# jviquerat/beacon

Measured on AMD Instinct MI355X. Metric: aggregate env steps/sec, rayleigh-v0 batch=512/GPU 128x64, higher is better.
Workload: dtype f32

## Files before the change

beacon_amd/build.py:

```python
import fcntl
import glob
import hashlib
import os
import shutil
import subprocess
from concurrent.futures import ThreadPoolExecutor

PKG = os.path.dirname(os.path.abspath(__file__))
CSRC = os.path.join(PKG, "csrc")
INC = os.path.join(os.path.dirname(PKG), "include")
LIB = os.path.join(PKG, "libbeacon_hip.so")
OBJ = os.path.join(PKG, "csrc", "_obj")
ARCH = "gfx950"
FLAGS = ["-O3", "-std=c++17", "-fPIC", "--offload-arch=" + ARCH, "-fvisibility=hidden",
         "-fgpu-rdc" if False else "-fno-gpu-rdc", "-Wall", "-Wno-unused-function",
         "-Wno-unused-variable", "-Wno-unused-but-set-variable"]


FILE_FLAGS = {"ns2d_fast.hip": ["-fno-slp-vectorize", "-ffp-contract=on", "-O2"],
              "ns2d_fast_f64.hip": ["-fno-slp-vectorize", "-ffp-contract=on"],
              "ns2d_fast2.hip": ["-fno-slp-vectorize", "-ffp-contract=on", "-mllvm", "-amdgpu-disable-unclustered-high-rp-reschedule",
                                 "-mllvm", "-amdgpu-sdwa-peephole=0"],
              "ns2d_fast_prm.hip": ["-fno-slp-vectorize", "-ffp-contract=on", "-O2"],
              "ns2d_fast_prm_f64.hip": ["-fno-slp-vectorize", "-ffp-contract=on"],
              "ns2d_fast2_prm.hip": ["-fno-slp-vectorize", "-ffp-contract=on", "-mllvm", "-amdgpu-disable-unclustered-high-rp-reschedule",
                                     "-mllvm", "-amdgpu-sdwa-peephole=0"],
              "env1d_f64.hip": ["-ffp-contract=off"],
              "shkadov_warm_f64.hip": ["-ffp-contract=off"],
              "ode_f64.hip": ["-ffp-contract=off"],
              "rollout.hip": ["-ffp-contract=off"],
              "render.hip": ["-ffp-contract=off", "-fhip-fp32-correctly-rounded-divide-sqrt"]}


JIT_FLAGS = ["-fno-slp-vectorize", "-ffp-contract=on"]


def hipcc():
    for c in (os.environ.get("HIPCC"), shutil.which("hipcc"), "/opt/rocm/bin/hipcc"):
        if c and os.path.exists(c):
            return c
    return None


def sources():
    return sorted(glob.glob(os.path.join(CSRC, "*.hip")))


def _deps():
    return (sources() + glob.glob(os.path.join(CSRC, "*.h")) + glob.glob(os.path.join(CSRC, "*.inc")) +
            [f for f in glob.glob(os.path.join(INC, "*.h")) if os.path.basename(f) not in ("beacon_actor.h", "beacon_learner.h")])


# ... 81 lines not shown
```

beacon_amd/csrc/bcn_dpp.h:

```cpp
#pragma once
#include "bcn_common.h"

namespace bcn_dpp {

template <int CTRL, int RM, int BM, bool BC>
__device__ __forceinline__ float dpp(float oldv, float v) {
  return __builtin_bit_cast(float, __builtin_amdgcn_update_dpp(__builtin_bit_cast(int, oldv),
                                                               __builtin_bit_cast(int, v), CTRL, RM, BM, BC));
}
template <int CTRL, int RM, int BM, bool BC>
__device__ __forceinline__ double dpp(double oldv, double v) {
  const long long o = __builtin_bit_cast(long long, oldv), s = __builtin_bit_cast(long long, v);
  const int lo = __builtin_amdgcn_update_dpp((int)o, (int)s, CTRL, RM, BM, BC);
  const int hi = __builtin_amdgcn_update_dpp((int)(o >> 32), (int)(s >> 32), CTRL, RM, BM, BC);
  return __builtin_bit_cast(double, ((long long)hi << 32) | (unsigned int)lo);
}
template <typename real> __device__ __forceinline__ real from_below(real oldv, real v) { return dpp<0x138, 0xf, 0xf, false>(oldv, v); }
template <typename real> __device__ __forceinline__ real from_above(real oldv, real v) { return dpp<0x130, 0xf, 0xf, false>(oldv, v); }

__device__ __forceinline__ float add_above_below(float acc, float c) {
  float t, r;
  asm("s_nop 1\n\t"
      "v_add_f32_dpp %0, %2, %3 wave_shl:1 row_mask:0xf bank_mask:0xf bound_ctrl:1\n\t"
      "v_add_f32_dpp %1, %2, %0 wave_shr:1 row_mask:0xf bank_mask:0xf bound_ctrl:1"
// ... 41 lines not shown
__device__ __forceinline__ real wave_sum_lane63(real s) {
  s = row16_sum(s);
  s += dpp<0x142, 0xa, 0xf, false>(real(0), s);
  s += dpp<0x143, 0xc, 0xf, false>(real(0), s);
  return s;
}
__device__ __forceinline__ float bcn_fmax(float a, float b) { return __builtin_fmaxf(a, b); }
__device__ __forceinline__ double bcn_fmax(double a, double b) { return __builtin_fmax(a, b); }
template <typename real>
__device__ __forceinline__ real row16_max(real s) {
  s = bcn_fmax(s, dpp<0x111, 0xf, 0xf, true>(real(0), s));
  s = bcn_fmax(s, dpp<0x112, 0xf, 0xf, true>(real(0), s));
  s = bcn_fmax(s, dpp<0x114, 0xf, 0xf, true>(real(0), s));
  s = bcn_fmax(s, dpp<0x118, 0xf, 0xf, true>(real(0), s));
  return s;
}
template <typename real>
__device__ __forceinline__ real wave_max_lane63(real s) {
  s = row16_max(s);
  s = bcn_fmax(s, dpp<0x142, 0xa, 0xf, false>(real(0), s));
  s = bcn_fmax(s, dpp<0x143, 0xc, 0xf, false>(real(0), s));
  return s;
}
__device__ __forceinline__ float read_lane(float v, int l) {
  return __builtin_bit_cast(float, __builtin_amdgcn_readlane(__builtin_bit_cast(int, v), l));
}
__device__ __forceinline__ double read_lane(double v, int l) {
  const long long s = __builtin_bit_cast(long long, v);
  const int lo = __builtin_amdgcn_readlane((int)s, l), hi = __builtin_amdgcn_readlane((int)(s >> 32), l);
  return __builtin_bit_cast(double, ((long long)hi << 32) | (unsigned int)lo);
}

}
```

beacon_amd/csrc/capi.hip:

```cpp
#include <math.h>
#include <stdarg.h>
#include <stddef.h>

#include <new>
#include <vector>

#include "env1d.h"
#include "ns2d.h"
#include "ns2d_builtin.h"
#include "ns2d_geom.h"
#include "ns2d_sched.h"
#include "ode_env.h"
#include "params.h"
#include "snapshot.h"
#include "episode.h"
#include "shkadov_jets.h"
#include "normalize.h"
#include "rollout.h"
#include "render.h"

static thread_local char g_err[512] = "";

__attribute__((visibility("default"))) void bcn_set_error(const char* fmt, ...) {
  va_list ap;
// ... 210 lines not shown
  }
  typedef int (*plugin_prm_fn)(const void*, int, void*, const void*);
  plugin_prm_fn plugin_prm = nullptr;
  int set_fast_plugin_params(void* fn) override {
    if (fn && !plugin) { bcn_set_error("bcn_set_fast_plugin_params: the handle has no kernel plugin (bcn_set_fast_plugin comes first)"); return BCN_ERR_ARG; }
    plugin_prm = reinterpret_cast<plugin_prm_fn>(fn);
    host.launched = nullptr;
    return BCN_OK;
  }
  NS2DHost host;
  const real* prm = nullptr;
  int params_kernel = 0;
  void use_params(const void* table) override { prm = static_cast<const real*>(table); host.launched = nullptr; }
  bool prm_fast() const {
    return prm && params_kernel == 1 && variant == 1 && (plugin ? plugin_prm != nullptr : ns2d_fast_supported_prm<real>(a));
  }
  const char* kernel_name() const override {
    if (prm && !prm_fast()) return "ns2d_generic_step";
    return host.launched ? host.launched : (variant == 1 ? "ns2d_fast_step" : "ns2d_generic_step");
  }
  int launch(hipStream_t s) {
    a.host = &host;
    if (prm) {
      if (prm_fast()) {
        const int rc = plugin ? plugin_prm(&a, batch, s, prm) : ns2d_launch_fast_prm<real>(a, batch, s, prm);
        if (rc != BCN_ERR_UNSUPPORTED) return rc;
      }
      return ns2d_launch_generic_prm<real>(a, batch, s, prm);
    }
    if (variant == 1 && plugin) {
      const int rc = plugin(&a, batch, s);
      if (rc != BCN_ERR_UNSUPPORTED) return rc;
      return ns2d_launch_generic<real>(a, batch, s);
    }
    if (variant == 1) return ns2d_launch_fast<real>(a, batch, s);
    return ns2d_launch_generic<real>(a, batch, s);
  }
};

template <typename real>
void ns2d_common(NS2DArgs<real>& a, int nx, int ny, double dx, double dy, double dt, double tol) {
  a.nx = nx; a.ny = ny; a.sx = nx + 2; a.ncell = (nx + 2) * (ny + 2);
  a.dt = (real)dt; a.rdx = (real)(1.0 / dx); a.rdy = (real)(1.0 / dy);
  a.rdx2 = (real)(1.0 / (dx * dx)); a.rdy2 = (real)(1.0 / (dy * dy));
  const double den = dx * dx + dy * dy;
  a.cx = (real)(0.5 * dy * dy / den);
  a.cy = (real)(0.5 * dx * dx / den);
  a.cb = (real)(0.5 * dx * dx * dy * dy / den / dt);
  a.tol = (real)tol;
}

template <typename real>
int make_rayleigh(const bcn_rayleigh_cfg* c, int batch, int dtype, int device, bcn_env_t* out) {
  return make_env<NS2DEnv<real>>(BCN_RAYLEIGH, batch, dtype, device, snap_cfg_hash<bcn_rayleigh_cfg, 12, 9>(c), out, [c](NS2DEnv<real>* e) {
    NS2DArgs<real>& a = e->a;
    ns2d_common(a, c->nx, c->ny, c->dx, c->dy, c->dt, c->tol);
    a.kind = 0; a.ndt_act = c->ndt_act; a.n_act = c->n_act; a.itmax = c->itmax;
    a.n_sgts = c->n_sgts; a.nx_sgts = c->nx_sgts;
    a.nxo = c->nx_obs_pts; a.nyo = c->ny_obs_pts; a.nx_obs = c->nx_obs; a.ny_obs = c->ny_obs;
    a.n_obs_steps = c->n_obs_steps; a.n_obs = 3 * c->n_obs_steps * c->nx_obs_pts * c->ny_obs_pts;
    a.kmom = (real)bcn_rayleigh_kmom(c->pr, c->ra);
    a.ksc = (real)bcn_rayleigh_ksc(c->pr, c->ra);
    e->prm_cfg[0] = c->ra; e->prm_aux[0] = c->pr;
    a.Tc = (real)c->Tc; a.Th = (real)c->Th; a.C = (real)c->C;
    a.rwd_scale = (real)(1.0 / (0.5 * c->dy * c->nx));
    e->n_obs = a.n_obs; e->n_act = c->n_sgts; e->ndt_act = a.ndt_act;
// ... 1168 lines not shown
```

beacon_amd/csrc/jit/ns2d_jit.hip:

```cpp
#if defined(BCN_JIT_PRM) && BCN_JIT_PRM
#define BCN_PRM_KERNELS 1
#endif
#if BCN_JIT_ROWS == 1 && BCN_JIT_KIND != 0
#error "ns2d_fast_impl.h (one row per lane, ny <= 64) implements the rayleigh boundary conditions only: mixing needs BCN_JIT_ROWS=2"
#endif
#if BCN_JIT_ROWS == 1
#include "../ns2d_fast_impl.h"
#elif BCN_JIT_ROWS == 2
#include "../ns2d_fast2_impl.h"
#else
#include "../ns2d_fast4_impl.h"
#endif

#ifndef BCN_JIT_GF
#define BCN_JIT_GF 0
#endif

extern "C" {

#ifdef BCN_PRM_KERNELS
#define BCN_JIT_TABLE , static_cast<const BCN_JIT_REAL*>(table)
__attribute__((visibility("default"))) int bcn_jit_launch(const void*, int, void*) {
  bcn_set_error("kernel plugin built with BCN_JIT_PRM: it holds the table-reading kernels only (bcn_jit_launch_prm)");
  return BCN_ERR_UNSUPPORTED;
}
__attribute__((visibility("default"))) int bcn_jit_launch_prm(const void* args, int batch, void* stream, const void* table) {
#else
#define BCN_JIT_TABLE
__attribute__((visibility("default"))) int bcn_jit_launch(const void* args, int batch, void* stream) {
#endif
#ifdef BCN_JIT_BREAK
#ifndef BCN_JIT_BREAK_EPS
#define BCN_JIT_BREAK_EPS 3e-4
#endif
  NS2DArgs<BCN_JIT_REAL> a = *static_cast<const NS2DArgs<BCN_JIT_REAL>*>(args);
#if BCN_JIT_BREAK == 2
  a.dt *= BCN_JIT_REAL(1.0 + BCN_JIT_BREAK_EPS);
#else
  a.dt *= BCN_JIT_REAL(1.5);
// ... 5 lines not shown
    bcn_set_error("kernel plugin built for %dx%d kind %d, handle is %dx%d kind %d", BCN_JIT_NX, BCN_JIT_NY, BCN_JIT_KIND,
                  a.nx, a.ny, a.kind);
    return BCN_ERR_ARG;
  }
#if BCN_JIT_ROWS == 1
  return launch_fast<BCN_JIT_REAL, BCN_JIT_NX, BCN_JIT_NY, BCN_JIT_R, BCN_JIT_KIND, BCN_JIT_GF>(a, batch, static_cast<hipStream_t>(stream) BCN_JIT_TABLE);
#elif BCN_JIT_ROWS == 2
  return launch_fast2<BCN_JIT_REAL, BCN_JIT_NX, BCN_JIT_NY, BCN_JIT_R, BCN_JIT_KIND, BCN_JIT_GF>(a, batch, static_cast<hipStream_t>(stream) BCN_JIT_TABLE);
#else
  return launch_fast4<BCN_JIT_REAL, BCN_JIT_NX, BCN_JIT_NY, BCN_JIT_R, BCN_JIT_RPL, BCN_JIT_KIND>(a, batch, static_cast<hipStream_t>(stream) BCN_JIT_TABLE);
#endif
}

__attribute__((visibility("default"))) size_t bcn_jit_scratch_elems(void) {
#if BCN_JIT_ROWS == 1
  return FastGeom<BCN_JIT_NX, BCN_JIT_NY, BCN_JIT_R, BCN_JIT_GF>::scratch_elems();
#elif BCN_JIT_ROWS == 2
  return Fast2Geom<BCN_JIT_NX, BCN_JIT_NY, BCN_JIT_R, BCN_JIT_GF>::scratch_elems();
#else
  return 0;
#endif
}

__attribute__((visibility("default"))) size_t bcn_jit_lds_bytes(void) {
#if BCN_JIT_ROWS == 1
  return FastGeom<BCN_JIT_NX, BCN_JIT_NY, BCN_JIT_R, BCN_JIT_GF>::lds_bytes<BCN_JIT_REAL>();
#elif BCN_JIT_ROWS == 2
  return Fast2Geom<BCN_JIT_NX, BCN_JIT_NY, BCN_JIT_R, BCN_JIT_GF>::lds_elems() * sizeof(BCN_JIT_REAL);
#else
  return (size_t)Fast4Geom<BCN_JIT_NX, BCN_JIT_NY, BCN_JIT_R, BCN_JIT_RPL>::lds_elems(sizeof(BCN_JIT_REAL)) * sizeof(BCN_JIT_REAL);
#endif
}

}
```

beacon_amd/csrc/ns2d.h:

```cpp
#pragma once
#include "bcn_common.h"

struct NS2DHost {
  const char* launched = nullptr;
  int sched_tail = 0;
  int generic_nt = 0;
};

template <typename real>
struct NS2DArgs {
  int nx, ny, sx, ncell;
  int ndt_act, n_act, itmax;
  int kind;
  int n_sgts, nx_sgts;
  int nxo, nyo, nx_obs, ny_obs, n_obs_steps, n_obs;
  int i_min, i_max, j_min, j_max;
  real dt, rdx, rdy, rdx2, rdy2;
  real kmom;
  real ksc;
  real cx, cy, cb;
  real tol;
  real Tc, Th, C, u_max, ref_c, C0;
  real rwd_scale;
  real *u, *v, *p, *S, *us, *vs;
// ... 13 lines not shown
  int32_t* sweeps;
  const real* init_fields;
  const uint8_t* mask;
  int work_in_lds;
  int it_begin, it_end;
  int first_chunk, last_chunk;
  const int32_t* order;
  int32_t* order_out;
  int32_t* sweeps_int;
  void* sched_ctl;
  unsigned long long* cyc;
  size_t sched_bytes;
  int sched_q;
  int sched_nbig = 0;
  int conv_plan = 1;
  int plan_overshoot = 0;
  int spec_start = 0;
  int verify_conv = 0;
  int sched_mode = -1;
  int sched_grid = 0, sched_q_user = 0, lpt_min_batch = 0;
  NS2DHost* host;
  real* fscr;
  size_t fscr_stride;
  int transport_iter = 0;
  float slow_l2lc[2] = {0.f, 0.f};
  float slow_cl[2] = {__builtin_inff(), __builtin_inff()};
};

template <typename real> int ns2d_launch_generic(const NS2DArgs<real>& a, int batch, hipStream_t s);
template <typename real> int ns2d_launch_reset(const NS2DArgs<real>& a, int batch, hipStream_t s);
size_t ns2d_generic_lds_bytes(int ncell, size_t esz);
template <typename real> bool ns2d_fast_supported(const NS2DArgs<real>& a);
template <typename real> int ns2d_launch_fast(const NS2DArgs<real>& a, int batch, hipStream_t s);
template <typename real> size_t ns2d_fast_scratch_elems(const NS2DArgs<real>& a);
template <typename real> bool ns2d_fast2_supported(const NS2DArgs<real>& a);
template <typename real> size_t ns2d_fast2_scratch_elems(const NS2DArgs<real>& a);
template <typename real> int ns2d_launch_fast2(const NS2DArgs<real>& a, int batch, hipStream_t s);
```

beacon_amd/csrc/ns2d_fast_impl.h:

```cpp
#pragma once
#include <stdlib.h>

#include <type_traits>

#include "bcn_dpp.h"
#include "ns2d.h"
#include "ns2d_cells.h"
#include "ns2d_device.h"
#include "ns2d_geom.h"
#include "ns2d_prm.h"
#include "ns2d_sched.h"




namespace {

using namespace bcn_dpp;

template <int NX, int NY, int R, int GF = 0>
struct FastGeom {
  static constexpr bcn_geom::Rows1 g{NX, NY, R, GF};
  static_assert(g.shape_ok(), "one row per lane: ny <= 64 (lanes run along y), at most 16 waves, at least 3 columns each");
  static constexpr int NW = g.nw();
  static constexpr int RL = g.rl();
  static constexpr int NT = g.threads();
  static constexpr int SY = g.sy();
  static constexpr int SX = g.sx();
  static constexpr int DEADPAD = g.deadpad();
  static constexpr int SZ = g.sz();
  static constexpr int PD = g.pd();
  static constexpr int XC = g.xc();
  static constexpr int EXCH = g.exch();
  static constexpr int SCHED_WORDS = g.sched_words();
  static constexpr int MISC = g.misc();
  static constexpr int FRONT = g.front();
  static constexpr int BACK = g.back();
  static constexpr int FRONTG = g.frontg();
  static constexpr int MISCA = g.misca();
  static constexpr size_t base_elems() { return g.base_elems(); }
  static constexpr size_t SCR = g.scr();
  template <typename real> static constexpr bool offload() { return g.offload(sizeof(real)); }
  template <typename real> static constexpr size_t lds_bytes() { return g.lds_bytes(sizeof(real)); }
  static constexpr size_t scratch_elems() { return g.scratch_elems(); }
};

typedef float v2f __attribute__((ext_vector_type(2)));
// ... 461 lines not shown
      const real a1q = (lane < NW) ? exch[((xb * NW + (lane < NW ? lane : 0)) * XC + 1) * 64] : real(0);
      const real a1 = read_lane(row16_sum<real>(a1q), 15);
      if (tid == 0) slow_k[0] = (real)(0.5f * __log2f(3.f * (float)a1 / (float)A.tol));
      xb ^= 1;
    } else if (A.conv_plan == 3) {
      real a1p = 0;
#pragma unroll
      for (int k = 0; k < R; k++) a1p += nb[k] * nb[k];
      const real a1w = wave_sum_lane63<real>(a1p);
      if (lane == 63) errp[(xb ^ 1) * 64 + w] = a1w;
      __syncthreads();
      const real a1 = read_lane(row16_sum<real>(errp[(xb ^ 1) * 64 + (lane & 15)]), 15);
      if (tid == 0) slow_k[0] = (real)(0.5f * __log2f(3.f * (float)a1 / (float)A.tol));
    }

    BCN_PH(1)
    const unsigned long long cyc_j0 = __builtin_amdgcn_s_memtime();
    auto cell = [&](real c, real e, real wv, real nbk) -> real {
      const real q = cBy * c + nbk;
      real ph;
      if constexpr (EQ && std::is_same<real, float>::value) {
        ph = jacobi_cell_eq(c, e, wv, nbk, cx, cBy);
      } else if (EQ) {
        real sum = e + wv;
        sum = add_above_below(sum, c);
        ph = cx * sum + q;
      } else {
        const real ns = dpp<0x130, 0xf, 0xf, true>(real(0), c) + dpp<0x138, 0xf, 0xf, true>(real(0), c);
        ph = cx * (e + wv) + (cy * ns + q);
      }
      if (NY < 64) ph *= actf;
      return ph;
    };
    real hW = 0, hE = 0;
    real hW1r, hW2r, hE1r, hE2r;
    int itp;
    real phA[R], phB[R];
    bool finalB;
    const real tolL0 = (A.conv_plan == 3) ? A.tol * real(BCN_CONV_GUARD) : A.tol;
    const float l2tol_u = __log2f((float)A.tol * 1.02f), l2tol_w = __log2f((float)tolL0 * 1.003f);
    constexpr int JMAX = 256;
#ifdef BCN_DBG_NCHK
    int nchk = 0;
#define BCN_NCHK_INC nchk++;
#else
#define BCN_NCHK_INC
#endif
#ifdef BCN_STAMP
    const unsigned long long st0 = __builtin_amdgcn_s_memtime();
#endif
    for (;;) {
    hW1r = 0; hW2r = 0; hE1r = 0; hE2r = 0;
    itp = 0;
#pragma unroll
    for (int k = 0; k < R; k++) phA[k] = 0;
    finalB = false;
    real tolL = tolL0;
    int k_prev = -1;
    float l2u_prev = 0, l2w_prev = 0;
    int skip_left = 0;
    const int plan = (A.conv_plan == 3) ? (__builtin_amdgcn_readfirstlane((int)prev_sweeps[1]) != 0 ? 1 : 2) : A.conv_plan;
#define BCN_CELLS(SRC, DST)                                                                  \
      _Pragma("unroll") for (int k = 1; k < R - 1; k++) DST[k] = cell(SRC[k], SRC[k + 1], SRC[k - 1], nb[k]); \
         \
      __builtin_amdgcn_sched_barrier(0);                                                     \
      hW = (w > 0) ? hW1r : SRC[0];                                                          \
      hE = (w < NW - 1) ? hE1r : SRC[R - 1];                                                 \
      const real p0 = cell(SRC[0], SRC[1], hW, nb[0]);                                       \
      const real pl = cell(SRC[R - 1], hE, SRC[R - 2], nb[R - 1]);                           \
      DST[0] = p0;                                                                           \
      DST[R - 1] = pl;                                                                       \
       \
      if constexpr (DEADC) DST[DEADC ? RL : 0] = lastw ? DST[DEADC ? RL - 1 : 0] : DST[DEADC ? RL : 0]; \
      BCN_PUBLISH(DST)
#define BCN_PUBLISH(DST)                                                                     \
      exl(xb, w, 0) = DST[0];                                                                \
      exl(xb, w, XL) = DST[R - 1];                                                           \
      if constexpr (XC == 4) { exl(xb, w, 1) = DST[1]; exl(xb, w, 2) = DST[R - 2]; }
#define BCN_HALO_READS                                                                       \
      hW1r = exl(xb, wm, XL);                                                                \
      hE1r = exl(xb, wp, 0);                                                                 \
      if constexpr (XC == 4) { hW2r = exl(xb, wm, 2); hE2r = exl(xb, wp, 1); }               \
      xb ^= 1;
#define BCN_SWEEP_END                                                                        \
      __syncthreads();                                                                       \
      itp++;                                                                                 \
      BCN_HALO_READS
#define BCN_FAST(SRC, DST) { BCN_CELLS(SRC, DST) BCN_SWEEP_END }
#define BCN_FAST2X(X, Y)                                                                     \
    {                                                                                        \
      _Pragma("unroll") for (int k = 1; k < R - 1; k++) Y[k] = cell(X[k], X[k + 1], X[k - 1], nb[k]); \
      __builtin_amdgcn_sched_barrier(0);                                                     \
      const real xw1 = (w > 0) ? hW1r : X[0], xe1 = (w < NW - 1) ? hE1r : X[R - 1];          \
      Y[0] = cell(X[0], X[1], xw1, nb[0]);                                                   \
      Y[R - 1] = cell(X[R - 1], xe1, X[R - 2], nb[R - 1]);                                   \
      real yw = cell(hW1r, X[0], hW2r, nbW), ye = cell(hE1r, hE2r, X[R - 1], nbE);           \
      yw = (w > 0) ? yw : Y[0];                                                              \
      ye = (w < NW - 1) ? ye : Y[R - 1];                                                     \
      __builtin_amdgcn_sched_barrier(0);                                                     \
                                   \
      X[0] = cell(Y[0], Y[1], yw, nb[0]);                                                    \
      X[1] = cell(Y[1], Y[2], Y[0], nb[1]);                                                  \
      X[R - 2] = cell(Y[R - 2], Y[R - 1], Y[R - 3], nb[R - 2]);                              \
      X[R - 1] = cell(Y[R - 1], ye, Y[R - 2], nb[R - 1]);                                    \
      hW = yw; hE = ye;                                                                      \
      BCN_PUBLISH(X)                                                                         \
      __builtin_amdgcn_sched_barrier(0);                                                     \
      _Pragma("unroll") for (int k = 2; k < R - 2; k++) X[k] = cell(Y[k], Y[k + 1], Y[k - 1], nb[k]); \
      __syncthreads();                                                                       \
      itp += 2;                                                                              \
      BCN_HALO_READS                                                                         \
    }
#define BCN_CHECK(SRC, DST, DST_IS_B)                                                        \
    {                                                                                        \
      BCN_CELLS(SRC, DST)                                                                    \
      BCN_NCHK_INC                                                                           \
      real acc = 0;                                                                          \
      _Pragma("unroll") for (int k = 1; k < R - 1; k++) {                                    \
        real d = DST[k] - SRC[k];                                                            \
        if (DEADC && k >= RL) d = lastw ? real(0) : d;    \
        acc += d * d;                                                                        \
      }                                                                                      \
      real pI = wl * acc;                                                                    \
      if constexpr (DEADC) { const real de = DST[DEADC ? RL - 1 : 0] - SRC[DEADC ? RL - 1 : 0]; pI += fEl * (de * de); } \
      const real d0 = p0 - SRC[0], dl = pl - SRC[R - 1];                                     \
      const real part = pI + cW * (d0 * d0) + cE * (dl * dl);                                \
      const real tot63 = wave_sum_lane63<real>(part);                                        \
      if (lane == 63) errp[xb * 64 + w] = tot63;                                             \
      if (plan == 1) {    \
        const real totu63 = wave_sum_lane63<real>(acc + d0 * d0 + (lastw ? real(0) : dl * dl)); \
        if (lane == 63) errp[xb * 64 + 16 + w] = totu63;                                     \
      }                                                                                      \
      __syncthreads();                                                                       \
      itp++;                                                                                 \
                                       \
      const real epart = errp[xb * 64 + (lane & 31)];                                        \
      BCN_HALO_READS                                                                         \
      const real esum = row16_sum<real>(epart);                                              \
      const real err = read_lane(esum, 15);                                                  \
       \
      const bool amb = SPEC && skip_left == -2 && plan == 1 && !(read_lane(esum, 31) > A.tol * real(1.02)); \
       \
// ... 8 lines not shown
      if (SPEC) skip_left = skip_left < 0 ? 0 : skip_left;                                   \
      n = 0;                                                                                 \
      if (skip_left > 0) {                                                                   \
        skip_left--;                                                                         \
      } else if (plan > 0) {                \
        const float l2u = (plan == 1) ? __log2f((float)read_lane(esum, 31)) : 0.f; \
        const float l2w = __log2f((float)err);                                               \
        int j = 0;                                                                           \
        if (k_prev >= 0) {                                                                   \
          const float rg = 1.f / (float)(itp - 1 - k_prev);                                  \
          if (plan == 1) {                                                            \
            const float room_u = l2u - l2tol_u, rho_u = (l2u - l2u_prev) * rg;               \
            j = ns2d_plan_steps(room_u, rho_u, JMAX);                                        \
          } else {                                                                           \
            float l2tl = l2tol_w;                                                            \
            if (A.conv_plan == 3) {    \
            const float g = ns2d_slow_guard<real>(slow_k, itp);                                                                              \
              tolL = A.tol * (real)g;                                                        \
              l2tl = __log2f((float)tolL * 1.003f);                                          \
            }                                                                                \
            const float room_w = l2w - l2tl, rho_w = (l2w - l2w_prev) * rg;                  \
            const int jw = ns2d_plan_steps(room_w, rho_w, JMAX);                             \
            j = ns2d_plan_trim(jw, A.plan_overshoot);                                        \
          }                                                                                  \
        }                                                                                    \
        j = __builtin_amdgcn_readfirstlane(j);                                               \
        l2u_prev = l2u; l2w_prev = l2w; k_prev = itp - 1;                                    \
        if (A.verify_conv) skip_left = j; else n = j;                                        \
      }                                                                                      \
    }
#define BCN_CHECK2X(X, Y)                                                                    \
    {                                                                                        \
      const int itp0 = itp;                                                                  \
      _Pragma("unroll") for (int k = 1; k < R - 1; k++) Y[k] = cell(X[k], X[k + 1], X[k - 1], nb[k]); \
      __builtin_amdgcn_sched_barrier(0);                                                     \
      const real xw1 = (w > 0) ? hW1r : X[0], xe1 = (w < NW - 1) ? hE1r : X[R - 1];          \
      Y[0] = cell(X[0], X[1], xw1, nb[0]);                                                   \
      Y[R - 1] = cell(X[R - 1], xe1, X[R - 2], nb[R - 1]);                                   \
      real yw = cell(hW1r, X[0], hW2r, nbW), ye = cell(hE1r, hE2r, X[R - 1], nbE);           \
      yw = (w > 0) ? yw : Y[0];                                                              \
      ye = (w < NW - 1) ? ye : Y[R - 1];                                                     \
      BCN_NCHK_INC BCN_NCHK_INC                                                              \
      real acc1 = 0;                                                                         \
      _Pragma("unroll") for (int k = 1; k < R - 1; k++) { const real d = Y[k] - X[k]; acc1 += d * d; } \
      const real d10 = Y[0] - X[0], d1l = Y[R - 1] - X[R - 1];                               \
      const real part1 = wl * acc1 + cW * (d10 * d10) + cE * (d1l * d1l);                    \
      const real upart1 = acc1 + d10 * d10 + d1l * d1l;                                      \
      __builtin_amdgcn_sched_barrier(0);                                                     \
      X[0] = cell(Y[0], Y[1], yw, nb[0]);                                                    \
      X[1] = cell(Y[1], Y[2], Y[0], nb[1]);                                                  \
      X[R - 2] = cell(Y[R - 2], Y[R - 1], Y[R - 3], nb[R - 2]);                              \
      X[R - 1] = cell(Y[R - 1], ye, Y[R - 2], nb[R - 1]);                                    \
      hW = yw; hE = ye;                                                                      \
      BCN_PUBLISH(X)                                                                         \
      __builtin_amdgcn_sched_barrier(0);                                                     \
      _Pragma("unroll") for (int k = 2; k < R - 2; k++) X[k] = cell(Y[k], Y[k + 1], Y[k - 1], nb[k]); \
      real acc2 = 0;                                                                         \
      _Pragma("unroll") for (int k = 1; k < R - 1; k++) { const real d = X[k] - Y[k]; acc2 += d * d; } \
      const real d20 = X[0] - Y[0], d2l = X[R - 1] - Y[R - 1];                               \
      const real part2 = wl * acc2 + cW * (d20 * d20) + cE * (d2l * d2l);                    \
      const real t1_63 = wave_sum_lane63<real>(part1), t2_63 = wave_sum_lane63<real>(part2); \
      if (lane == 63) { errp[xb * 64 + w] = t1_63; errp[xb * 64 + 16 + w] = t2_63; }         \
      if (plan == 1) {    \
        const real u1_63 = wave_sum_lane63<real>(upart1);                                    \
        const real u2_63 = wave_sum_lane63<real>(acc2 + d20 * d20 + d2l * d2l);              \
        if (lane == 63) { errp[xb * 64 + 32 + w] = u1_63; errp[xb * 64 + 48 + w] = u2_63; }  \
      }                                                                                      \
      __syncthreads();                                                                       \
      itp += 2;                                                                              \
      const real epart = errp[xb * 64 + lane];                                               \
      BCN_HALO_READS                                                                         \
      const real esum = row16_sum<real>(epart);                                              \
      const real err1 = read_lane(esum, 15), err2 = read_lane(esum, 31);                     \
       \
      const bool ov1 = itp - 1 > A.itmax, ov2 = itp > A.itmax;                               \
      const bool pass1 = ov1 || !(err1 > A.tol), pass2 = ov2 || !(err2 > A.tol);             \
       \
      const bool amb = SPEC && skip_left == -2 && plan == 1 && !(read_lane(esum, 47) > A.tol * real(1.02)); \
       \
      const bool unv = plan >= 2 && !A.verify_conv && itp0 > 0 && k_prev != itp0 && !(err1 > tolL); \
      if (pass1 || pass2 || amb || unv) {                                                    \
        const bool ovf = ov1 || (ov2 && (err1 > A.tol));                                     \
        if (ovf) status |= BCN_ST_ITMAX;                                                     \
        if (!ovf && skip_left > (pass1 ? 0 : 1)) status |= BCN_ST_PLAN;    \
        if (SPEC) skip_left = (skip_left == -2 && !ovf) ? -1 : 0;                            \
        finalB = pass1;                                                                      \
        itp -= pass1 ? 1 : 0;                                                                \
         \
        hW1r = pass1 ? yw : hW1r;                                                            \
// ... 55 lines not shown
        for (; n > 0; n -= 2) BCN_FAST2X(phA, phB)
      }
    } else {
    for (;;) {
      int n;
      BCN_CHECK(phA, phB, true)
      if (n == 0) {
        BCN_CHECK(phB, phA, false)
        n &= ~1;
      } else {
        BCN_FAST(phB, phA)
        n = (n - 1) & ~1;
      }
      if (SPEC && XC != 4 && itp == 2 && A.spec_start > 0 && plan > 0 && !A.verify_conv) {
        const int prev = __builtin_amdgcn_readfirstlane((int)prev_sweeps[0]);
        const int ns = ((prev * (A.spec_start <= 16 ? A.spec_start : 6)) >> 3) - 2;
        if (prev >= 16 && ns > n) { n = ns & ~1; skip_left = -2; }
      }
      if (n > A.itmax - itp) n = (A.itmax - itp > 0 ? A.itmax - itp : 0) & ~1;
      if constexpr (XC == 4) {
        for (; n > 0; n -= 2) BCN_FAST2X(phA, phB)
      } else {
        for (; n > 0; n -= 2) {
          BCN_FAST(phA, phB)
          BCN_FAST(phB, phA)
        }
      }
    }
    late_stop = itp >= 2 && k_prev != itp - 2;
    }
#undef BCN_CHECK2X
#undef BCN_CHECK
#undef BCN_FAST2X
#undef BCN_HALO_READS
#undef BCN_PUBLISH
#undef BCN_FAST
#undef BCN_SWEEP_END
#undef BCN_CELLS
    {
      const bool toofar = SPEC && skip_left == -1;
      const bool late = plan >= 2 && !toofar && late_stop && !(status & BCN_ST_ITMAX);
      if (late && tid == 0) prev_sweeps[2] += 1;
      if (!(toofar || (late && A.conv_plan == 3))) {
        if (tid == 0) { prev_sweeps[0] = SPEC ? (real)itp : real(0); prev_sweeps[1] = 0; }
        break;
      }
      if (tid == 0) { prev_sweeps[0] = 0; prev_sweeps[1] = toofar ? real(0) : real(1); prev_sweeps[3] += 1; }
      __syncthreads();
    }
    }
    if (finalB) {
#pragma unroll
      for (int k = 0; k < R; k++) phA[k] = phB[k];
    }
    hW = hW1r;
#ifdef BCN_STAMP
    {
      const unsigned long long st1 = __builtin_amdgcn_s_memtime();
      const int cps = (int)((st1 - st0) / (unsigned long long)(itp > 0 ? itp : 1));
      if (A.sweeps && tid == 0) A.sweeps[(size_t)b * A.ndt_act + it] = itp | (cps << 16);
    }
#elif defined(BCN_DBG_NCHK)
    if (A.sweeps && tid == 0) A.sweeps[(size_t)b * A.ndt_act + it] = itp | (nchk << 16);
#else
    if (A.sweeps && tid == 0) A.sweeps[(size_t)b * A.ndt_act + it] = itp;
#endif

    cyc_j += __builtin_amdgcn_s_memtime() - cyc_j0;
    asm volatile("" : "+v"(j));
    BCN_PH(2)
#pragma unroll
// ... 168 lines not shown
```

beacon_amd/csrc/ns2d_fast_prm.hip:

```cpp
#define BCN_PRM_KERNELS 1
#include "params.h"
#include "ns2d_fast.hip"
```

Baseline: 29580.

## Emit Jacobi cell runs as batched inline asm blocks with split tail sync

```diff
diff --git a/beacon_amd/build.py b/beacon_amd/build.py
--- a/beacon_amd/build.py
+++ b/beacon_amd/build.py
@@ -18,6 +18,7 @@
 
 
 FILE_FLAGS = {"ns2d_fast.hip": ["-fno-slp-vectorize", "-ffp-contract=on", "-O2"],
+              "ns2d_fast_runs.hip": ["-fno-slp-vectorize", "-ffp-contract=on", "-O2"],
               "ns2d_fast_f64.hip": ["-fno-slp-vectorize", "-ffp-contract=on"],
               "ns2d_fast2.hip": ["-fno-slp-vectorize", "-ffp-contract=on", "-mllvm", "-amdgpu-disable-unclustered-high-rp-reschedule",
                                  "-mllvm", "-amdgpu-sdwa-peephole=0"],
diff --git a/beacon_amd/csrc/bcn_dpp.h b/beacon_amd/csrc/bcn_dpp.h
--- a/beacon_amd/csrc/bcn_dpp.h
+++ b/beacon_amd/csrc/bcn_dpp.h
@@ -97,3 +97,5 @@
 }
 
 }
+
+#include "bcn_jacobi_cells.h"
diff --git a/beacon_amd/csrc/bcn_jacobi_cells.h b/beacon_amd/csrc/bcn_jacobi_cells.h
--- /dev/null
+++ b/beacon_amd/csrc/bcn_jacobi_cells.h
@@ -0,0 +1,72 @@
+#pragma once
+
+#define BCN_RUN_CELL0 "v_add_f32 %[t], %[a2], %[a0]\n\t" "s_nop 1\n\t" "v_add_f32_dpp %[u], %[a1], %[t] wave_shl:1 row_mask:0xf bank_mask:0xf bound_ctrl:1\n\t" "v_add_f32_dpp %[t], %[a1], %[u] wave_shr:1 row_mask:0xf bank_mask:0xf bound_ctrl:1\n\t" "v_fma_f32 %[q], %[cBy], %[a1], %[n0]\n\t" "v_fma_f32 %[d0], %[cx], %[t], %[q]\n\t"
+#define BCN_RUN_CELL1 "v_add_f32 %[t], %[a3], %[a1]\n\t" "s_nop 1\n\t" "v_add_f32_dpp %[u], %[a2], %[t] wave_shl:1 row_mask:0xf bank_mask:0xf bound_ctrl:1\n\t" "v_add_f32_dpp %[t], %[a2], %[u] wave_shr:1 row_mask:0xf bank_mask:0xf bound_ctrl:1\n\t" "v_fma_f32 %[q], %[cBy], %[a2], %[n1]\n\t" "v_fma_f32 %[d1], %[cx], %[t], %[q]\n\t"
+#define BCN_RUN_CELL2 "v_add_f32 %[t], %[a4], %[a2]\n\t" "s_nop 1\n\t" "v_add_f32_dpp %[u], %[a3], %[t] wave_shl:1 row_mask:0xf bank_mask:0xf bound_ctrl:1\n\t" "v_add_f32_dpp %[t], %[a3], %[u] wave_shr:1 row_mask:0xf bank_mask:0xf bound_ctrl:1\n\t" "v_fma_f32 %[q], %[cBy], %[a3], %[n2]\n\t" "v_fma_f32 %[d2], %[cx], %[t], %[q]\n\t"
+#define BCN_RUN_CELL3 "v_add_f32 %[t], %[a5], %[a3]\n\t" "s_nop 1\n\t" "v_add_f32_dpp %[u], %[a4], %[t] wave_shl:1 row_mask:0xf bank_mask:0xf bound_ctrl:1\n\t" "v_add_f32_dpp %[t], %[a4], %[u] wave_shr:1 row_mask:0xf bank_mask:0xf bound_ctrl:1\n\t" "v_fma_f32 %[q], %[cBy], %[a4], %[n3]\n\t" "v_fma_f32 %[d3], %[cx], %[t], %[q]\n\t"
+#define BCN_RUN_CELL4 "v_add_f32 %[t], %[a6], %[a4]\n\t" "s_nop 1\n\t" "v_add_f32_dpp %[u], %[a5], %[t] wave_shl:1 row_mask:0xf bank_mask:0xf bound_ctrl:1\n\t" "v_add_f32_dpp %[t], %[a5], %[u] wave_shr:1 row_mask:0xf bank_mask:0xf bound_ctrl:1\n\t" "v_fma_f32 %[q], %[cBy], %[a5], %[n4]\n\t" "v_fma_f32 %[d4], %[cx], %[t], %[q]\n\t"
+#define BCN_RUN_CELL5 "v_add_f32 %[t], %[a7], %[a5]\n\t" "s_nop 1\n\t" "v_add_f32_dpp %[u], %[a6], %[t] wave_shl:1 row_mask:0xf bank_mask:0xf bound_ctrl:1\n\t" "v_add_f32_dpp %[t], %[a6], %[u] wave_shr:1 row_mask:0xf bank_mask:0xf bound_ctrl:1\n\t" "v_fma_f32 %[q], %[cBy], %[a6], %[n5]\n\t" "v_fma_f32 %[d5], %[cx], %[t], %[q]\n\t"
+#define BCN_RUN_CELL6 "v_add_f32 %[t], %[a8], %[a6]\n\t" "s_nop 1\n\t" "v_add_f32_dpp %[u], %[a7], %[t] wave_shl:1 row_mask:0xf bank_mask:0xf bound_ctrl:1\n\t" "v_add_f32_dpp %[t], %[a7], %[u] wave_shr:1 row_mask:0xf bank_mask:0xf bound_ctrl:1\n\t" "v_fma_f32 %[q], %[cBy], %[a7], %[n6]\n\t" "v_fma_f32 %[d6], %[cx], %[t], %[q]\n\t"
+#define BCN_ANY_CELL0 "v_add_f32 %[t], %[e0], %[w0]\n\t" "s_nop 1\n\t" "v_add_f32_dpp %[u], %[c0], %[t] wave_shl:1 row_mask:0xf bank_mask:0xf bound_ctrl:1\n\t" "v_add_f32_dpp %[t], %[c0], %[u] wave_shr:1 row_mask:0xf bank_mask:0xf bound_ctrl:1\n\t" "v_fma_f32 %[q], %[cBy], %[c0], %[n0]\n\t" "v_fma_f32 %[d0], %[cx], %[t], %[q]\n\t"
+#define BCN_ANY_CELL1 "v_add_f32 %[t], %[e1], %[w1]\n\t" "s_nop 1\n\t" "v_add_f32_dpp %[u], %[c1], %[t] wave_shl:1 row_mask:0xf bank_mask:0xf bound_ctrl:1\n\t" "v_add_f32_dpp %[t], %[c1], %[u] wave_shr:1 row_mask:0xf bank_mask:0xf bound_ctrl:1\n\t" "v_fma_f32 %[q], %[cBy], %[c1], %[n1]\n\t" "v_fma_f32 %[d1], %[cx], %[t], %[q]\n\t"
+#define BCN_ANY_CELL2 "v_add_f32 %[t], %[e2], %[w2]\n\t" "s_nop 1\n\t" "v_add_f32_dpp %[u], %[c2], %[t] wave_shl:1 row_mask:0xf bank_mask:0xf bound_ctrl:1\n\t" "v_add_f32_dpp %[t], %[c2], %[u] wave_shr:1 row_mask:0xf bank_mask:0xf bound_ctrl:1\n\t" "v_fma_f32 %[q], %[cBy], %[c2], %[n2]\n\t" "v_fma_f32 %[d2], %[cx], %[t], %[q]\n\t"
+#define BCN_ANY_CELL3 "v_add_f32 %[t], %[e3], %[w3]\n\t" "s_nop 1\n\t" "v_add_f32_dpp %[u], %[c3], %[t] wave_shl:1 row_mask:0xf bank_mask:0xf bound_ctrl:1\n\t" "v_add_f32_dpp %[t], %[c3], %[u] wave_shr:1 row_mask:0xf bank_mask:0xf bound_ctrl:1\n\t" "v_fma_f32 %[q], %[cBy], %[c3], %[n3]\n\t" "v_fma_f32 %[d3], %[cx], %[t], %[q]\n\t"
+
+namespace bcn_dpp {
+
+#define BCN_CELLS_TMP [t] "=&v"(t), [u] "=&v"(u), [q] "=&v"(q)
+#define BCN_RUN_O1 BCN_CELLS_TMP, [d0] "=&v"(d[0])
+#define BCN_RUN_O2 BCN_RUN_O1, [d1] "=&v"(d[1])
+#define BCN_RUN_O3 BCN_RUN_O2, [d2] "=&v"(d[2])
+#define BCN_RUN_O4 BCN_RUN_O3, [d3] "=&v"(d[3])
+#define BCN_RUN_O5 BCN_RUN_O4, [d4] "=&v"(d[4])
+#define BCN_RUN_O6 BCN_RUN_O5, [d5] "=&v"(d[5])
+#define BCN_RUN_O7 BCN_RUN_O6, [d6] "=&v"(d[6])
+#define BCN_RUN_I1 [cx] "s"(cx), [cBy] "v"(cBy), [a0] "v"(a[0]), [a1] "v"(a[1]), [a2] "v"(a[2]), [n0] "v"(n[0])
+#define BCN_RUN_I2 BCN_RUN_I1, [a3] "v"(a[3]), [n1] "v"(n[1])
+#define BCN_RUN_I3 BCN_RUN_I2, [a4] "v"(a[4]), [n2] "v"(n[2])
+#define BCN_RUN_I4 BCN_RUN_I3, [a5] "v"(a[5]), [n3] "v"(n[3])
+#define BCN_RUN_I5 BCN_RUN_I4, [a6] "v"(a[6]), [n4] "v"(n[4])
+#define BCN_RUN_I6 BCN_RUN_I5, [a7] "v"(a[7]), [n5] "v"(n[5])
+#define BCN_RUN_I7 BCN_RUN_I6, [a8] "v"(a[8]), [n6] "v"(n[6])
+
+template <int M>
+__device__ __forceinline__ void jacobi_run_eq(float* __restrict__ d, const float* __restrict__ a, const float* __restrict__ n, float cx, float cBy) {
+  static_assert(M >= 1 && M <= 7, "3 M + 7 operands, 30 at the most");
+  float t, u, q;
+  if constexpr (M == 1) asm(BCN_RUN_CELL0 : BCN_RUN_O1 : BCN_RUN_I1);
+  if constexpr (M == 2) asm(BCN_RUN_CELL0 BCN_RUN_CELL1 : BCN_RUN_O2 : BCN_RUN_I2);
+  if constexpr (M == 3) asm(BCN_RUN_CELL0 BCN_RUN_CELL1 BCN_RUN_CELL2 : BCN_RUN_O3 : BCN_RUN_I3);
+  if constexpr (M == 4) asm(BCN_RUN_CELL0 BCN_RUN_CELL1 BCN_RUN_CELL2 BCN_RUN_CELL3 : BCN_RUN_O4 : BCN_RUN_I4);
+  if constexpr (M == 5) asm(BCN_RUN_CELL0 BCN_RUN_CELL1 BCN_RUN_CELL2 BCN_RUN_CELL3 BCN_RUN_CELL4 : BCN_RUN_O5 : BCN_RUN_I5);
+  if constexpr (M == 6) asm(BCN_RUN_CELL0 BCN_RUN_CELL1 BCN_RUN_CELL2 BCN_RUN_CELL3 BCN_RUN_CELL4 BCN_RUN_CELL5 : BCN_RUN_O6 : BCN_RUN_I6);
+  if constexpr (M == 7) asm(BCN_RUN_CELL0 BCN_RUN_CELL1 BCN_RUN_CELL2 BCN_RUN_CELL3 BCN_RUN_CELL4 BCN_RUN_CELL5 BCN_RUN_CELL6 : BCN_RUN_O7 : BCN_RUN_I7);
+}
+constexpr bool jacobi_runs_fit(int r) { return r - 4 <= 3 || r - 4 >= 8; }
+constexpr int jacobi_run_len(int n) { return (n + (n + 6) / 7 - 1) / ((n + 6) / 7); }
+template <int K0, int K1>
+__device__ __forceinline__ void jacobi_range_eq(float* __restrict__ dst, const float* __restrict__ src, const float* __restrict__ nb, float cx, float cBy) {
+  if constexpr (K1 > K0) {
+    constexpr int M = jacobi_run_len(K1 - K0);
+    jacobi_run_eq<M>(dst + K0, src + K0 - 1, nb + K0, cx, cBy);
+    jacobi_range_eq<K0 + M, K1>(dst, src, nb, cx, cBy);
+  }
+}
+
+#define BCN_ANY_O(i) , [d##i] "=&v"(d##i)
+#define BCN_ANY_I(i) , [c##i] "v"(c##i), [e##i] "v"(e##i), [w##i] "v"(w##i), [n##i] "v"(n##i)
+__device__ __forceinline__ void jacobi_cells_eq(float& d0, float& d1, float c0, float e0, float w0, float n0, float c1, float e1, float w1, float n1,
+                                                float cx, float cBy) {
+  float t, u, q;
+  asm(BCN_ANY_CELL0 BCN_ANY_CELL1 : BCN_CELLS_TMP BCN_ANY_O(0) BCN_ANY_O(1) : [cx] "s"(cx), [cBy] "v"(cBy) BCN_ANY_I(0) BCN_ANY_I(1));
+}
+__device__ __forceinline__ void jacobi_cells_eq(float& d0, float& d1, float& d2, float& d3, float c0, float e0, float w0, float n0, float c1, float e1,
+                                                float w1, float n1, float c2, float e2, float w2, float n2, float c3, float e3, float w3, float n3,
+                                                float cx, float cBy) {
+  float t, u, q;
+  asm(BCN_ANY_CELL0 BCN_ANY_CELL1 BCN_ANY_CELL2 BCN_ANY_CELL3
+      : BCN_CELLS_TMP BCN_ANY_O(0) BCN_ANY_O(1) BCN_ANY_O(2) BCN_ANY_O(3)
+      : [cx] "s"(cx), [cBy] "v"(cBy) BCN_ANY_I(0) BCN_ANY_I(1) BCN_ANY_I(2) BCN_ANY_I(3));
+}
+
+}
diff --git a/beacon_amd/csrc/capi.hip b/beacon_amd/csrc/capi.hip
--- a/beacon_amd/csrc/capi.hip
+++ b/beacon_amd/csrc/capi.hip
@@ -266,6 +266,9 @@
       const int rc = plugin(&a, batch, s);
       if (rc != BCN_ERR_UNSUPPORTED) return rc;
       return ns2d_launch_generic<real>(a, batch, s);
+    }
+    if constexpr (std::is_same<real, float>::value) {
+      if (variant == 1 && ns2d_fast_runs_supported(a)) return ns2d_launch_fast_runs(a, batch, s);
     }
     if (variant == 1) return ns2d_launch_fast<real>(a, batch, s);
     return ns2d_launch_generic<real>(a, batch, s);
diff --git a/beacon_amd/csrc/jit/ns2d_jit.hip b/beacon_amd/csrc/jit/ns2d_jit.hip
--- a/beacon_amd/csrc/jit/ns2d_jit.hip
+++ b/beacon_amd/csrc/jit/ns2d_jit.hip
@@ -5,6 +5,7 @@
 #error "ns2d_fast_impl.h (one row per lane, ny <= 64) implements the rayleigh boundary conditions only: mixing needs BCN_JIT_ROWS=2"
 #endif
 #if BCN_JIT_ROWS == 1
+#define BCN_JACOBI_RUNS 1
 #include "../ns2d_fast_impl.h"
 #elif BCN_JIT_ROWS == 2
 #include "../ns2d_fast2_impl.h"
@@ -76,4 +77,12 @@
 #endif
 }
 
+__attribute__((visibility("default"))) int bcn_jit_cell_runs(void) {
+#if BCN_JIT_ROWS == 1
+  return std::is_same<BCN_JIT_REAL, float>::value && bcn_dpp::jacobi_runs_fit(BCN_JIT_R) ? 1 : 0;
+#else
+  return 0;
+#endif
 }
+
+}
diff --git a/beacon_amd/csrc/ns2d.h b/beacon_amd/csrc/ns2d.h
--- a/beacon_amd/csrc/ns2d.h
+++ b/beacon_amd/csrc/ns2d.h
@@ -69,6 +69,8 @@
 size_t ns2d_generic_lds_bytes(int ncell, size_t esz);
 template <typename real> bool ns2d_fast_supported(const NS2DArgs<real>& a);
 template <typename real> int ns2d_launch_fast(const NS2DArgs<real>& a, int batch, hipStream_t s);
+bool ns2d_fast_runs_supported(const NS2DArgs<float>& a);
+int ns2d_launch_fast_runs(const NS2DArgs<float>& a, int batch, hipStream_t s);
 template <typename real> size_t ns2d_fast_scratch_elems(const NS2DArgs<real>& a);
 template <typename real> bool ns2d_fast2_supported(const NS2DArgs<real>& a);
 template <typename real> size_t ns2d_fast2_scratch_elems(const NS2DArgs<real>& a);
diff --git a/beacon_amd/csrc/ns2d_fast_impl.h b/beacon_amd/csrc/ns2d_fast_impl.h
--- a/beacon_amd/csrc/ns2d_fast_impl.h
+++ b/beacon_amd/csrc/ns2d_fast_impl.h
@@ -13,6 +13,10 @@
 
 
 
+
+#ifndef BCN_JACOBI_RUNS
+#define BCN_JACOBI_RUNS 0
+#endif
 
 namespace {
 
@@ -540,6 +544,38 @@
       if (NY < 64) ph *= actf;
       return ph;
     };
+    constexpr bool RUNS = BCN_JACOBI_RUNS && EQ && std::is_same<real, float>::value && jacobi_runs_fit(R0);
+#define BCN_RANGE(DST, SRC, K0, K1)                                                          \
+      if constexpr (RUNS) {                                                                  \
+        jacobi_range_eq<K0, K1>(DST, SRC, nb, cx, cBy);                                      \
+        if (NY < 64) { _Pragma("unroll") for (int k = K0; k < K1; k++) DST[k] *= actf; }     \
+      } else {                                                                               \
+        _Pragma("unroll") for (int k = K0; k < K1; k++) DST[k] = cell(SRC[k], SRC[k + 1], SRC[k - 1], nb[k]); \
+      }
+#define BCN_EDGE4(X, Y)                                                                      \
+      real yw, ye;                                                                           \
+      if constexpr (RUNS) {                                                                  \
+        jacobi_cells_eq(Y[0], Y[R - 1], yw, ye, X[0], X[1], xw1, nb[0], X[R - 1], xe1, X[R - 2], nb[R - 1], \
+                        hW1r, X[0], hW2r, nbW, hE1r, hE2r, X[R - 1], nbE, cx, cBy);          \
+        if (NY < 64) { Y[0] *= actf; Y[R - 1] *= actf; yw *= actf; ye *= actf; }             \
+      } else {                                                                               \
+        Y[0] = cell(X[0], X[1], xw1, nb[0]);                                                 \
+        Y[R - 1] = cell(X[R - 1], xe1, X[R - 2], nb[R - 1]);                                 \
+        yw = cell(hW1r, X[0], hW2r, nbW); ye = cell(hE1r, hE2r, X[R - 1], nbE);              \
+      }                                                                                      \
+      yw = (w > 0) ? yw : Y[0];                                                              \
+      ye = (w < NW - 1) ? ye : Y[R - 1];
+#define BCN_XCHG4(X, Y)                                                                      \
+      if constexpr (RUNS && R >= 4) {                                                        \
+        jacobi_cells_eq(X[0], X[1], X[R - 2], X[R - 1], Y[0], Y[1], yw, nb[0], Y[1], Y[2], Y[0], nb[1], \
+                        Y[R - 2], Y[R - 1], Y[R - 3], nb[R - 2], Y[R - 1], ye, Y[R - 2], nb[R - 1], cx, cBy); \
+        if (NY < 64) { X[0] *= actf; X[1] *= actf; X[R - 2] *= actf; X[R - 1] *= actf; }     \
+      } else {                                                                               \
+        X[0] = cell(Y[0], Y[1], yw, nb[0]);                                                  \
+        X[1] = cell(Y[1], Y[2], Y[0], nb[1]);                                                \
+        X[R - 2] = cell(Y[R - 2], Y[R - 1], Y[R - 3], nb[R - 2]);                            \
+        X[R - 1] = cell(Y[R - 1], ye, Y[R - 2], nb[R - 1]);                                  \
+      }
     real hW = 0, hE = 0;
     real hW1r, hW2r, hE1r, hE2r;
     int itp;
@@ -569,13 +605,19 @@
     int skip_left = 0;
     const int plan = (A.conv_plan == 3) ? (__builtin_amdgcn_readfirstlane((int)prev_sweeps[1]) != 0 ? 1 : 2) : A.conv_plan;
 #define BCN_CELLS(SRC, DST)                                                                  \
-      _Pragma("unroll") for (int k = 1; k < R - 1; k++) DST[k] = cell(SRC[k], SRC[k + 1], SRC[k - 1], nb[k]); \
+      BCN_RANGE(DST, SRC, 1, R - 1)                                                          \
          \
       __builtin_amdgcn_sched_barrier(0);                                                     \
       hW = (w > 0) ? hW1r : SRC[0];                                                          \
       hE = (w < NW - 1) ? hE1r : SRC[R - 1];                                                 \
-      const real p0 = cell(SRC[0], SRC[1], hW, nb[0]);                                       \
-      const real pl = cell(SRC[R - 1], hE, SRC[R - 2], nb[R - 1]);                           \
+      real p0, pl;                                                                           \
+      if constexpr (RUNS) {                                                                  \
+        jacobi_cells_eq(p0, pl, SRC[0], SRC[1], hW, nb[0], SRC[R - 1], hE, SRC[R - 2], nb[R - 1], cx, cBy); \
+        if (NY < 64) { p0 *= actf; pl *= actf; }                                             \
+      } else {                                                                               \
+        p0 = cell(SRC[0], SRC[1], hW, nb[0]);                                                \
+        pl = cell(SRC[R - 1], hE, SRC[R - 2], nb[R - 1]);                                    \
+      }                                                                                      \
       DST[0] = p0;                                                                           \
       DST[R - 1] = pl;                                                                       \
        \
@@ -595,27 +637,31 @@
       itp++;                                                                                 \
       BCN_HALO_READS
 #define BCN_FAST(SRC, DST) { BCN_CELLS(SRC, DST) BCN_SWEEP_END }
+#define BCN_TAIL2(X, Y)                                                                      \
+      if constexpr (RUNS && R - 4 >= 8) {                                                    \
+        constexpr int KB = 2 + (R - 4) / 2;                                                  \
+        BCN_RANGE(X, Y, 2, KB)                                                               \
+        __builtin_amdgcn_sched_barrier(0);                                                   \
+        __syncthreads();                                                                     \
+        __builtin_amdgcn_sched_barrier(0);                                                   \
+        BCN_RANGE(X, Y, KB, R - 2)                                                           \
+      } else {                                                                               \
+        BCN_RANGE(X, Y, 2, R - 2)                                                            \
+        __syncthreads();                                                                     \
+      }
 #define BCN_FAST2X(X, Y)                                                                     \
     {                                                                                        \
-      _Pragma("unroll") for (int k = 1; k < R - 1; k++) Y[k] = cell(X[k], X[k + 1], X[k - 1], nb[k]); \
+      BCN_RANGE(Y, X, 1, R - 1)                                                              \
       __builtin_amdgcn_sched_barrier(0);                                                     \
       const real xw1 = (w > 0) ? hW1r : X[0], xe1 = (w < NW - 1) ? hE1r : X[R - 1];          \
-      Y[0] = cell(X[0], X[1], xw1, nb[0]);                                                   \
-      Y[R - 1] = cell(X[R - 1], xe1, X[R - 2], nb[R - 1]);                                   \
-      real yw = cell(hW1r, X[0], hW2r, nbW), ye = cell(hE1r, hE2r, X[R - 1], nbE);           \
-      yw = (w > 0) ? yw : Y[0];                                                              \
-      ye = (w < NW - 1) ? ye : Y[R - 1];                                                     \
+      BCN_EDGE4(X, Y)                                                                        \
       __builtin_amdgcn_sched_barrier(0);                                                     \
                                    \
-      X[0] = cell(Y[0], Y[1], yw, nb[0]);                                                    \
-      X[1] = cell(Y[1], Y[2], Y[0], nb[1]);                                                  \
-      X[R - 2] = cell(Y[R - 2], Y[R - 1], Y[R - 3], nb[R - 2]);                              \
-      X[R - 1] = cell(Y[R - 1], ye, Y[R - 2], nb[R - 1]);                                    \
+      BCN_XCHG4(X, Y)                                                                        \
       hW = yw; hE = ye;                                                                      \
       BCN_PUBLISH(X)                                                                         \
       __builtin_amdgcn_sched_barrier(0);                                                     \
-      _Pragma("unroll") for (int k = 2; k < R - 2; k++) X[k] = cell(Y[k], Y[k + 1], Y[k - 1], nb[k]); \
-      __syncthreads();                                                                       \
+      BCN_TAIL2(X, Y)                                                                        \
       itp += 2;                                                                              \
       BCN_HALO_READS                                                                         \
     }
@@ -690,14 +736,10 @@
 #define BCN_CHECK2X(X, Y)                                                                    \
     {                                                                                        \
       const int itp0 = itp;                                                                  \
-      _Pragma("unroll") for (int k = 1; k < R - 1; k++) Y[k] = cell(X[k], X[k + 1], X[k - 1], nb[k]); \
+      BCN_RANGE(Y, X, 1, R - 1)                                                              \
       __builtin_amdgcn_sched_barrier(0);                                                     \
       const real xw1 = (w > 0) ? hW1r : X[0], xe1 = (w < NW - 1) ? hE1r : X[R - 1];          \
-      Y[0] = cell(X[0], X[1], xw1, nb[0]);                                                   \
-      Y[R - 1] = cell(X[R - 1], xe1, X[R - 2], nb[R - 1]);                                   \
-      real yw = cell(hW1r, X[0], hW2r, nbW), ye = cell(hE1r, hE2r, X[R - 1], nbE);           \
-      yw = (w > 0) ? yw : Y[0];                                                              \
-      ye = (w < NW - 1) ? ye : Y[R - 1];                                                     \
+      BCN_EDGE4(X, Y)                                                                        \
       BCN_NCHK_INC BCN_NCHK_INC                                                              \
       real acc1 = 0;                                                                         \
       _Pragma("unroll") for (int k = 1; k < R - 1; k++) { const real d = Y[k] - X[k]; acc1 += d * d; } \
@@ -705,14 +747,11 @@
       const real part1 = wl * acc1 + cW * (d10 * d10) + cE * (d1l * d1l);                    \
       const real upart1 = acc1 + d10 * d10 + d1l * d1l;                                      \
       __builtin_amdgcn_sched_barrier(0);                                                     \
-      X[0] = cell(Y[0], Y[1], yw, nb[0]);                                                    \
-      X[1] = cell(Y[1], Y[2], Y[0], nb[1]);                                                  \
-      X[R - 2] = cell(Y[R - 2], Y[R - 1], Y[R - 3], nb[R - 2]);                              \
-      X[R - 1] = cell(Y[R - 1], ye, Y[R - 2], nb[R - 1]);                                    \
+      BCN_XCHG4(X, Y)                                                                        \
       hW = yw; hE = ye;                                                                      \
       BCN_PUBLISH(X)                                                                         \
       __builtin_amdgcn_sched_barrier(0);                                                     \
-      _Pragma("unroll") for (int k = 2; k < R - 2; k++) X[k] = cell(Y[k], Y[k + 1], Y[k - 1], nb[k]); \
+      BCN_RANGE(X, Y, 2, R - 2)                                                              \
       real acc2 = 0;                                                                         \
       _Pragma("unroll") for (int k = 1; k < R - 1; k++) { const real d = X[k] - Y[k]; acc2 += d * d; } \
       const real d20 = X[0] - Y[0], d2l = X[R - 1] - Y[R - 1];                               \
@@ -834,11 +873,15 @@
 #undef BCN_CHECK2X
 #undef BCN_CHECK
 #undef BCN_FAST2X
+#undef BCN_TAIL2
 #undef BCN_HALO_READS
 #undef BCN_PUBLISH
 #undef BCN_FAST
 #undef BCN_SWEEP_END
 #undef BCN_CELLS
+#undef BCN_XCHG4
+#undef BCN_EDGE4
+#undef BCN_RANGE
     {
       const bool toofar = SPEC && skip_left == -1;
       const bool late = plan >= 2 && !toofar && late_stop && !(status & BCN_ST_ITMAX);
diff --git a/beacon_amd/csrc/ns2d_fast_prm.hip b/beacon_amd/csrc/ns2d_fast_prm.hip
--- a/beacon_amd/csrc/ns2d_fast_prm.hip
+++ b/beacon_amd/csrc/ns2d_fast_prm.hip
@@ -1,3 +1,4 @@
 #define BCN_PRM_KERNELS 1
+#define BCN_JACOBI_RUNS 1
 #include "params.h"
 #include "ns2d_fast.hip"
diff --git a/beacon_amd/csrc/ns2d_fast_runs.hip b/beacon_amd/csrc/ns2d_fast_runs.hip
--- /dev/null
+++ b/beacon_amd/csrc/ns2d_fast_runs.hip
@@ -0,0 +1,41 @@
+#define BCN_JACOBI_RUNS 1
+#include "ns2d_builtin.h"
+#include "ns2d_fast_impl.h"
+
+namespace {
+
+bool runs_pre(const NS2DArgs<float>& a) { return a.kind == 0 && a.n_sgts <= 64; }
+
+template <typename REAL, int R> constexpr bool runs_row() { return std::is_same<REAL, float>::value && jacobi_runs_fit(R); }
+
+}
+
+bool ns2d_fast_runs_supported(const NS2DArgs<float>& a) {
+#define BCN_ROW(REAL, NX, NY, R, KIND, GF) \
+  if (runs_row<REAL, R>() && BCN_BUILTIN_IS(float, a, REAL, NX, NY, KIND)) return runs_pre(a);
+  BCN_BUILTIN_FAST(BCN_ROW)
+#undef BCN_ROW
+  return false;
+}
+
+namespace {
+template <typename real>
+int launch_runs(const NS2DArgs<real>& a, int batch, hipStream_t s) {
+#define BCN_ROW(REAL, NX, NY, R, KIND, GF)                                                         \
+  if constexpr (std::is_same<real, REAL>::value && runs_row<REAL, R>()) {                     \
+    if (BCN_BUILTIN_IS(real, a, REAL, NX, NY, KIND) && runs_pre(a)) return launch_fast<REAL, NX, NY, R, KIND, GF>(a, batch, s); \
+  }
+  BCN_BUILTIN_FAST(BCN_ROW)
+#undef BCN_ROW
+  bcn_set_error("no register-resident kernel with cell runs for this grid");
+  return BCN_ERR_UNSUPPORTED;
+}
+}
+
+int ns2d_launch_fast_runs(const NS2DArgs<float>& a, int batch, hipStream_t s) { return launch_runs<float>(a, batch, s); }
+
+extern "C" __attribute__((visibility("default"))) int bcn_builtin_cell_runs(int nx, int ny) {
+  NS2DArgs<float> a{};
+  a.nx = nx; a.ny = ny; a.kind = 0; a.n_sgts = 1;
+  return ns2d_fast_runs_supported(a) ? 1 : 0;
+}
```

Measured after the change: 29940 (median of 6 runs). 1.01x the previous value.
